# ravenprotocol/ravnest

Hardware: AMD Instinct MI355X
Metric: samples/sec (whole node), BERT-base MLM pretraining (higher is better)
Workload: dtype bf16; 1 GPU; model=bert-base, global_batch=128, seq_len=512, parallelism=dp1, reduce_factor=4, optimizer=fused_adam

## Files before the change

### ravnest_amd/csrc/bindings.cpp

```cpp
#include <torch/extension.h>

#include <vector>

std::vector<at::Tensor> layernorm_fwd(at::Tensor x, at::Tensor w,
                                      at::Tensor b, double eps);
std::vector<at::Tensor> layernorm_bwd(at::Tensor dy, at::Tensor x,
                                      at::Tensor w, at::Tensor mean,
                                      at::Tensor rstd);
std::vector<at::Tensor> layernorm_add_fwd(at::Tensor a, at::Tensor b,
                                          at::Tensor w, at::Tensor bias,
                                          double eps);
std::vector<at::Tensor> layernorm_mx_fwd(at::Tensor x, at::Tensor w,
                                         at::Tensor b, double eps);
at::Tensor bias_gelu_fwd(at::Tensor x, at::Tensor bias);
std::vector<at::Tensor> bias_gelu_mx_fwd(at::Tensor x, at::Tensor bias);
at::Tensor bias_gelu_bwd(at::Tensor dy, at::Tensor x, at::Tensor bias);
at::Tensor colsum_bf16(at::Tensor x);
std::vector<at::Tensor> bias_gelu_bwd_db(at::Tensor dy, at::Tensor x,
                                         at::Tensor bias);
std::vector<at::Tensor> batchnorm_fwd(at::Tensor x, at::Tensor w,
                                      at::Tensor b, at::Tensor running_mean,
                                      at::Tensor running_var, bool training,
                                      double momentum, double eps);
std::vector<at::Tensor> batchnorm_bwd(at::Tensor dy, at::Tensor x,
// ... 29 lines not shown
                   at::Tensor ws, c10::optional<at::Tensor> bias);
at::Tensor mx_gemm2(at::Tensor xq, at::Tensor xs, at::Tensor wq,
                    at::Tensor ws, c10::optional<at::Tensor> bias);
at::Tensor mx_scale_probe(at::Tensor a, at::Tensor b, at::Tensor sa,
                          at::Tensor sb);
at::Tensor softmax_fwd(at::Tensor x);
at::Tensor softmax_bwd(at::Tensor dy, at::Tensor y);
std::vector<at::Tensor> maxpool2d_fwd(at::Tensor x, long K, long S, long P);
at::Tensor maxpool2d_bwd(at::Tensor dy, at::Tensor idx, long H, long W,
                         long K, long S, long P);
at::Tensor avgpool2d_fwd(at::Tensor x, long K, long S, long P,
                         bool include_pad);
at::Tensor avgpool2d_bwd(at::Tensor dy, long H, long W, long K, long S,
                         long P, bool include_pad);
at::Tensor global_avgpool_fwd(at::Tensor x);
at::Tensor global_avgpool_bwd(at::Tensor dy, long H, long W);
std::vector<at::Tensor> emb2_ln_fwd(at::Tensor ids, at::Tensor word,
                                    at::Tensor pos, at::Tensor w,
                                    at::Tensor b, double eps);
at::Tensor emb2_add_fwd(at::Tensor ids, at::Tensor word, at::Tensor pos);
std::vector<at::Tensor> emb2_bwd(at::Tensor dx, at::Tensor ids, long V,
                                 long P);
std::vector<at::Tensor> dropout_fwd(at::Tensor x, double p, int64_t seed,
                                    c10::optional<at::Tensor> seed_buf);
at::Tensor dropout_bwd(at::Tensor dy, at::Tensor mask, double p);
std::vector<at::Tensor> dropout_add_ln_fwd(at::Tensor z, at::Tensor a,
                                           at::Tensor w, at::Tensor bias,
                                           double eps, double p, int64_t seed,
                                           c10::optional<at::Tensor> seed_buf);
std::vector<at::Tensor> dropout_add_ln_bwd(at::Tensor dy, at::Tensor s,
                                           at::Tensor w, at::Tensor mean,
                                           at::Tensor rstd,
                                           at::Tensor maskbits, double p);
std::vector<at::Tensor> ce_fwd(at::Tensor logits, at::Tensor targets,
                               int64_t ignore_index);
at::Tensor ce_bwd(at::Tensor logits, at::Tensor targets, at::Tensor lse,
                  at::Tensor gscale, int64_t ignore_index);
std::vector<at::Tensor> mlm_head_fwd(at::Tensor h, at::Tensor W,
                                     at::Tensor b, at::Tensor targets,
                                     int64_t ignore_index);
std::vector<at::Tensor> mlm_head_bwd(at::Tensor dloss, at::Tensor logits_c,
                                     at::Tensor lse, at::Tensor hc,
                                     at::Tensor tc, at::Tensor pos,
                                     at::Tensor count, at::Tensor W);
std::tuple<at::Tensor, long, long> mt_build_table(
    std::vector<at::Tensor> ps, std::vector<at::Tensor> gs,
    std::vector<at::Tensor> ms, std::vector<at::Tensor> vs,
    std::vector<at::Tensor> masters);
std::tuple<at::Tensor, long, long> grad_build_table(
    std::vector<at::Tensor> gs);
void grad_sqnorm(at::Tensor table, long nchunks, long esize,
                 at::Tensor partials, long offset);
void grad_norm_finalize(at::Tensor partials, long n, at::Tensor stats,
                        double max_norm,
                        c10::optional<at::Tensor> max_norm_buf);
void scale_mt(at::Tensor table, long nchunks, long esize, at::Tensor gstats);
void fused_adam_graph(at::Tensor table, long nchunks, long esize,
                      at::Tensor lr_buf, double b1, double b2, double eps,
                      double wd, at::Tensor step_buf,
                      c10::optional<at::Tensor> gstats);
void fused_adam_table(at::Tensor table, long nchunks, long esize, double lr,
                      double b1, double b2, double eps, double wd, double bc1,
                      double bc2, c10::optional<at::Tensor> gstats);
void fused_sgd_table(at::Tensor table, long nchunks, long esize, double lr,
                     double momentum, double wd, bool nesterov,
                     c10::optional<at::Tensor> gstats);
// ... 34 lines not shown
        "fused LayerNorm fwd + MX fp8 quantisation of y: y, mean, rstd, q, "
        "s (bf16 x, hidden % 32 == 0)");
  m.def("bias_gelu_fwd", &bias_gelu_fwd, "fused bias+GELU fwd");
  m.def("bias_gelu_mx_fwd", &bias_gelu_mx_fwd,
        "fused bias+GELU fwd + MX fp8 quantisation of y: y, q, s (bf16 x, "
        "last dim % 32 == 0)");
  m.def("bias_gelu_bwd", &bias_gelu_bwd, "fused bias+GELU bwd");
  m.def("colsum_bf16", &colsum_bf16, "column sum bf16 -> fp32");
  m.def("bias_gelu_bwd_db", &bias_gelu_bwd_db,
        "fused bias+GELU bwd with in-pass bias-grad column reduction");
  m.def("batchnorm_fwd", &batchnorm_fwd, "fused BatchNorm2d fwd (NCHW)");
  m.def("batchnorm_bwd", &batchnorm_bwd, "fused BatchNorm2d bwd (NCHW)");
  m.def("batchnorm_relu_launch_constants", &batchnorm_relu_launch_constants,
        "(grid cap, block size, bytes per lane) of the BN+ReLU elementwise "
        "kernels");
  m.def("batchnorm_relu_fwd", &batchnorm_relu_fwd,
        "fused BatchNorm2d + [residual add] + ReLU fwd (NCHW)", py::arg("x"),
        py::arg("residual"), py::arg("w"), py::arg("b"),
        py::arg("running_mean"), py::arg("running_var"),
        py::arg("training"), py::arg("momentum"), py::arg("eps"));
  m.def("batchnorm_relu_bwd", &batchnorm_relu_bwd,
        "fused BatchNorm2d + [residual add] + ReLU bwd: dx, dw, db[, dr]");
  m.def("dropout_fwd", &dropout_fwd, "philox dropout fwd (replayable)",
        py::arg("x"), py::arg("p"), py::arg("seed"),
        py::arg("seed_buf") = py::none());
  m.def("dropout_bwd", &dropout_bwd, "dropout bwd");
  m.def("dropout_add_ln_fwd", &dropout_add_ln_fwd,
        "fused dropout + residual add + LayerNorm fwd (bf16, bit mask)",
        py::arg("z"), py::arg("a"), py::arg("w"), py::arg("bias"),
        py::arg("eps"), py::arg("p"), py::arg("seed"),
        py::arg("seed_buf") = py::none());
  m.def("dropout_add_ln_bwd", &dropout_add_ln_bwd,
        "fused dropout + residual add + LayerNorm bwd: dx, dz, dw, db");
  m.def("conv2d_fwd", &conv2d_fwd,
        "implicit-GEMM MFMA conv fwd (bf16 NCHW)", py::arg("x"),
        py::arg("w"), py::arg("bias") = py::none(), py::arg("st") = 1,
        py::arg("pad") = 0, py::arg("relu") = false);
  m.def("conv2d_dgrad", &conv2d_dgrad, "implicit-GEMM MFMA conv dgrad");
  m.def("conv2d_wgrad", &conv2d_wgrad, "implicit-GEMM MFMA conv wgrad");
  m.def("gemm_nt_bf16", &gemm_nt_bf16,
        "bf16 MFMA GEMM x @ W^T (256^2 8-phase, fused bias/GELU epilogue)",
        py::arg("a"), py::arg("b"), py::arg("bias") = py::none(),
        py::arg("epi") = 0);
  m.def("gemm_wgrad_bf16", &gemm_wgrad_bf16,
        "split-K wgrad dW = dy^T @ x (tr16 transpose reads, fp32 atomics)");
  m.def("gemm_nt_bf16_rows", &gemm_nt_bf16_rows,
        "gemm_nt_bf16 into the caller's C (row stride C.size(1)), rows "
        "below a device-side int32 limit only; epi 0 or 1",
        py::arg("a"), py::arg("b"), py::arg("bias"), py::arg("epi"),
        py::arg("c"), py::arg("row_limit"));
  m.def("gemm_wgrad_bf16_rows", &gemm_wgrad_bf16_rows,
        "gemm_wgrad_bf16 over rows [0, round_up(min(*row_bound, M), 64))",
        py::arg("dy"), py::arg("x"), py::arg("row_bound"));
  m.def("mx_quant", &mx_quant,
        "bf16 -> MX fp8 (e4m3 + per-32 e8m0 scales)");
  m.def("mx_gemm", &mx_gemm, "MX fp8 GEMM: x @ W^T, 32x32x64 scaled MFMA",
        py::arg("x"), py::arg("xs"), py::arg("w"), py::arg("ws"),
        py::arg("bias") = py::none());
  m.def("mx_gemm2", &mx_gemm2,
        "LDS-staged MX fp8 GEMM (256^2 4-phase, scaled 32x32x64 MFMA)",
        py::arg("xq"), py::arg("xs"), py::arg("wq"), py::arg("ws"),
        py::arg("bias") = py::none());
  m.def("mx_scale_probe", &mx_scale_probe,
        "per-lane scale-byte semantics probe");
  m.def("softmax_fwd", &softmax_fwd, "standalone softmax fwd (last dim)");
  m.def("softmax_bwd", &softmax_bwd, "standalone softmax bwd");
// ... 81 lines not shown
```

### ravnest_amd/csrc/dropout_ln.hip

```cpp
#include <torch/extension.h>
#include <ATen/hip/HIPContext.h>

#include <cstdint>

#include "common.h"

namespace {

typedef unsigned int u32x2 __attribute__((ext_vector_type(2)));
typedef __bf16 hwbf16x2 __attribute__((ext_vector_type(2)));
typedef float f32x2 __attribute__((ext_vector_type(2)));

DEVINL unsigned int pack2(float lo, float hi) {
  const f32x2 v = {lo, hi};
  return __builtin_bit_cast(unsigned int,
                            __builtin_convertvector(v, hwbf16x2));
}
DEVINL u32x2 pack4(const float f[4]) {
  u32x2 r;
  r[0] = pack2(f[0], f[1]);
  r[1] = pack2(f[2], f[3]);
  return r;
}
DEVINL void unpack4(u32x2 v, float f[4]) {
// ... 139 lines not shown
      }
    }
    const float rstd = rsqrtf(wave_sum(s2) / H + eps);
    if (lane == 0) {
      mean_out[row] = mean;
      rstd_out[row] = rstd;
    }

#pragma unroll
    for (int k = 0; k < VPL; ++k) {
      const int g = lane + WAVE * k;
      if (FULL || g < G) {
        float wk[4], bk[4];
        if constexpr (HOIST) {
#pragma unroll
          for (int j = 0; j < 4; ++j) {
            wk[j] = wv[k][j];
            bk[j] = bv[k][j];
          }
        } else {
          load_p4(w + 4 * g, wk);
          load_p4(bias + 4 * g, bk);
        }
        float o[4];
#pragma unroll
        for (int j = 0; j < 4; ++j)
          o[j] = (sv[k][j] - mean) * rstd * wk[j] + bk[j];
        *reinterpret_cast<u32x2*>(y + base + 4 * g) = pack4(o);
      }
    }
  }
}

template <typename PT, int VPL, bool FULL>
__global__ __launch_bounds__(BWD_THREADS)
__attribute__((amdgpu_waves_per_eu(VPL <= 3 ? 4 : 1)))
void dropout_add_ln_bwd_kernel(
    const bf16_t* __restrict__ dy, const bf16_t* __restrict__ s,
    const PT* __restrict__ w, const float* __restrict__ mean,
    const float* __restrict__ rstd,
    const unsigned char* __restrict__ maskbits, bf16_t* __restrict__ dx,
    bf16_t* __restrict__ dz, float* __restrict__ part, int H, long N,
    float scale) {
  extern __shared__ float red[];
  constexpr bool HOIST = VPL <= 4;
  constexpr int PV = HOIST ? VPL : 1;
  const int lane = threadIdx.x & (WAVE - 1);
  const int wid = threadIdx.x / WAVE;
  const int wpb = blockDim.x / WAVE;
  const long nwaves = (long)gridDim.x * wpb;
  const int G = H >> 2;

  float wv[PV][4];
  if constexpr (HOIST) {
#pragma unroll
    for (int k = 0; k < VPL; ++k) {
      const int g = lane + WAVE * k;
      if (FULL || g < G) load_p4(w + 4 * g, wv[k]);
    }
  }
  float accw[VPL][4], accb[VPL][4];
#pragma unroll
  for (int k = 0; k < VPL; ++k)
#pragma unroll
    for (int j = 0; j < 4; ++j) accw[k][j] = accb[k][j] = 0.f;

  for (long row = (long)blockIdx.x * wpb + wid; row < N; row += nwaves) {
    const long base = row * H;
    u32x2 vd[VPL], vx[VPL];
    unsigned int mb[VPL];
#pragma unroll
    for (int k = 0; k < VPL; ++k) {
      const int g = lane + WAVE * k;
      if (FULL || g < G) {
        vd[k] = *reinterpret_cast<const u32x2*>(dy + base + 4 * g);
        vx[k] = *reinterpret_cast<const u32x2*>(s + base + 4 * g);
        mb[k] = maskbits[(base >> 3) + (g >> 1)];
      }
    }
    const float mu = mean[row], rs = rstd[row];

    float gv[VPL][4], xh[VPL][4];
    float c1 = 0.f, c2 = 0.f;
#pragma unroll
    for (int k = 0; k < VPL; ++k) {
      const int g = lane + WAVE * k;
      if (FULL || g < G) {
        float wk[4];
        if constexpr (HOIST) {
#pragma unroll
          for (int j = 0; j < 4; ++j) wk[j] = wv[k][j];
        } else {
          load_p4(w + 4 * g, wk);
        }
        float df[4], xf[4];
        unpack4(vd[k], df);
        unpack4(vx[k], xf);
#pragma unroll
        for (int j = 0; j < 4; ++j) {
          const float d = df[j];
          const float xhat = (xf[j] - mu) * rs;
          const float gg = d * wk[j];
          c1 += gg * xhat;
          c2 += gg;
          accw[k][j] += d * xhat;
          accb[k][j] += d;
          gv[k][j] = gg;
          xh[k][j] = xhat;
        }
      }
    }
    c1 = wave_sum(c1) / H;
    c2 = wave_sum(c2) / H;

#pragma unroll
    for (int k = 0; k < VPL; ++k) {
      const int g = lane + WAVE * k;
      if (FULL || g < G) {
        const unsigned int nib = mb[k] >> ((lane & 1) * 4);
        float o[4];
#pragma unroll
        for (int j = 0; j < 4; ++j)
          o[j] = rs * (gv[k][j] - xh[k][j] * c1 - c2);
        const u32x2 ox = pack4(o);
        unpack4(ox, o);
#pragma unroll
        for (int j = 0; j < 4; ++j)
          o[j] = ((nib >> j) & 1) ? o[j] * scale : 0.f;
        *reinterpret_cast<u32x2*>(dx + base + 4 * g) = ox;
        *reinterpret_cast<u32x2*>(dz + base + 4 * g) = pack4(o);
      }
    }
  }

  for (int t = 0; t < wpb; ++t) {
    if (wid == t) {
#pragma unroll
      for (int k = 0; k < VPL; ++k) {
        const int g = lane + WAVE * k;
        if (FULL || g < G) {
#pragma unroll
          for (int j = 0; j < 4; ++j) {
            const int c = 4 * g + j;
            if (t == 0) {
              red[c] = accw[k][j];
              red[H + c] = accb[k][j];
            } else {
              red[c] += accw[k][j];
              red[H + c] += accb[k][j];
            }
          }
        }
      }
    }
    __syncthreads();
  }
  float* prow = part + (long)blockIdx.x * 2 * H;
  for (int i = threadIdx.x; i < 2 * H; i += blockDim.x) prow[i] = red[i];
}

template <typename PT>
__global__ __launch_bounds__(1024) void dropout_add_ln_bwd_finalize_kernel(
    const float* __restrict__ part, PT* __restrict__ dw, PT* __restrict__ db,
    int H, int nparts) {
  __shared__ float tile[32][33];
  const int c = threadIdx.x & 31;
  const int sl = threadIdx.x >> 5;
  const int col = blockIdx.x * 32 + c;
  float acc = 0.f;
  if (col < 2 * H) {
#pragma unroll 4
    for (int q = sl; q < nparts; q += 32)
      acc += part[(long)q * 2 * H + col];
  }
  tile[sl][c] = acc;
  __syncthreads();
  if (sl == 0 && col < 2 * H) {
    float t = 0.f;
#pragma unroll
    for (int i = 0; i < 32; ++i) t += tile[i][c];
    if (col < H)
      store_p1(dw + col, t);
    else
      store_p1(db + (col - H), t);
  }
}

template <typename K>
int resident_blocks(K kernel, int threads, size_t lds) {
  int per_cu = 0;
  hipError_t e = hipOccupancyMaxActiveBlocksPerMultiprocessor(
      &per_cu, kernel, threads, lds);
  int dev = 0, cus = 0;
  if (e == hipSuccess) e = hipGetDevice(&dev);
  if (e == hipSuccess)
    e = hipDeviceGetAttribute(&cus, hipDeviceAttributeMultiprocessorCount,
                              dev);
  TORCH_CHECK(e == hipSuccess && per_cu > 0 && cus > 0,
              "dropout_add_ln: occupancy query failed");
  return per_cu * cus;
}

template <typename PT, int VPL, bool FULL>
int fwd_resident_blocks() {
  static const int n = resident_blocks(
      dropout_add_ln_fwd_kernel<PT, VPL, FULL>, FWD_THREADS, 0);
  return n;
}
template <typename PT, int VPL, bool FULL>
int bwd_resident_blocks() {
  static const int n = resident_blocks(
      dropout_add_ln_bwd_kernel<PT, VPL, FULL>, BWD_THREADS,
      2 * VPL * 256 * sizeof(float));
  return n;
}

bool aligned8(const at::Tensor& t) {
  return reinterpret_cast<uintptr_t>(t.data_ptr()) % 8 == 0;
}
bool aligned16(const at::Tensor& t) {
  return reinterpret_cast<uintptr_t>(t.data_ptr()) % 16 == 0;
}

void check_common(const at::Tensor& x, const at::Tensor& w, const char* op) {
  TORCH_CHECK(x.is_cuda() && x.is_contiguous() &&
                  x.scalar_type() == at::kBFloat16 && x.dim() >= 1,
              op, ": bf16 contiguous device activations only");
  const long H = x.size(-1);
  TORCH_CHECK(H % 8 == 0 && H <= MAX_H && H > 0, op,
              ": hidden size must be a multiple of 8, at most ", MAX_H);
  TORCH_CHECK(w.is_cuda() && w.is_contiguous() && w.numel() == H &&
                  (w.scalar_type() == at::kFloat ||
                   w.scalar_type() == at::kBFloat16) &&
                  aligned16(w),
              op, ": LN parameters must be fp32 or bf16 of size H");
}

}

#define DAL_FULL(PT, VPL, LAUNCH)                                           \
  do {                                                                      \
    if (full_ && vpl_ == VPL) { LAUNCH(PT, VPL, true); }                    \
    else { LAUNCH(PT, VPL, false); }                                        \
  } while (0)
#define DAL_DISPATCH_VPL(PT, LAUNCH)                                        \
  do {                                                                      \
// ... 29 lines not shown
  auto maskbits = at::empty({N * H / 8}, a.options().dtype(at::kByte));
  if (N == 0) return {y, s_out, mean, rstd, maskbits};
  const float scale = 1.0f / (1.0f - (float)p);
  auto stream = c10::hip::getCurrentHIPStreamMasqueradingAsCUDA().stream();
  const int wpb = FWD_THREADS / WAVE;

#define DAL_LAUNCH_FWD(PT, VPL, FULL)                                       \
  do {                                                                      \
    const long want = (N + wpb - 1) / wpb;                                  \
    const int cap = fwd_resident_blocks<PT, VPL, FULL>();                   \
    dim3 grid((unsigned)std::min<long>(want, cap));                         \
    hipLaunchKernelGGL((dropout_add_ln_fwd_kernel<PT, VPL, FULL>), grid,    \
                       dim3(FWD_THREADS), 0, stream,                        \
                       reinterpret_cast<const bf16_t*>(z.data_ptr()),       \
                       reinterpret_cast<const bf16_t*>(a.data_ptr()),       \
                       reinterpret_cast<const PT*>(w.data_ptr()),           \
                       reinterpret_cast<const PT*>(bias.data_ptr()),        \
                       reinterpret_cast<bf16_t*>(y.data_ptr()),             \
                       reinterpret_cast<bf16_t*>(s_out.data_ptr()),         \
                       mean.data_ptr<float>(), rstd.data_ptr<float>(),      \
                       maskbits.data_ptr<unsigned char>(), H, N,            \
                       (float)eps, (float)p, scale,                         \
                       (unsigned long long)seed, sb);                       \
  } while (0)

  if (w.scalar_type() == at::kFloat)
    DAL_DISPATCH_VPL(float, DAL_LAUNCH_FWD);
  else
    DAL_DISPATCH_VPL(bf16_t, DAL_LAUNCH_FWD);
  HIP_CHECK_LAST();
  return {y, s_out, mean, rstd, maskbits};
}

std::vector<at::Tensor> dropout_add_ln_bwd(at::Tensor dy, at::Tensor s,
                                           at::Tensor w, at::Tensor mean,
                                           at::Tensor rstd,
                                           at::Tensor maskbits, double p) {
  check_common(s, w, "dropout_add_ln_bwd");
  check_common(dy, w, "dropout_add_ln_bwd");
  TORCH_CHECK(dy.sizes() == s.sizes() && aligned8(dy) && aligned8(s));
  const int H = s.size(-1);
  const long N = s.numel() / H;
  TORCH_CHECK(mean.is_cuda() && mean.scalar_type() == at::kFloat &&
              mean.is_contiguous() && mean.numel() == N);
  TORCH_CHECK(rstd.is_cuda() && rstd.scalar_type() == at::kFloat &&
              rstd.is_contiguous() && rstd.numel() == N);
  TORCH_CHECK(maskbits.is_cuda() && maskbits.scalar_type() == at::kByte &&
              maskbits.is_contiguous() && maskbits.numel() == N * H / 8);
  TORCH_CHECK(p > 0.0 && p < 1.0, "dropout_add_ln_bwd: p must be in (0, 1)");
  auto dx = at::empty_like(s);
  auto dz = at::empty_like(s);
  auto dw = at::empty({H}, w.options());
  auto db = at::empty({H}, w.options());
  if (N == 0) {
    dw.zero_();
    db.zero_();
    return {dx, dz, dw, db};
  }
  const float scale = 1.0f / (1.0f - (float)p);
  auto stream = c10::hip::getCurrentHIPStreamMasqueradingAsCUDA().stream();
  const int wpb = BWD_THREADS / WAVE;
  const size_t lds = 2 * (size_t)H * sizeof(float);

#define DAL_LAUNCH_BWD(PT, VPL, FULL)                                       \
  do {                                                                      \
    const long want = (N + wpb - 1) / wpb;                                  \
    const int nparts =                                                      \
        (int)std::min<long>(want, bwd_resident_blocks<PT, VPL, FULL>());    \
    auto part = at::empty({nparts, 2 * H}, s.options().dtype(at::kFloat));  \
    hipLaunchKernelGGL((dropout_add_ln_bwd_kernel<PT, VPL, FULL>),          \
                       dim3(nparts),                                        \
                       dim3(BWD_THREADS), lds, stream,                      \
                       reinterpret_cast<const bf16_t*>(dy.data_ptr()),      \
                       reinterpret_cast<const bf16_t*>(s.data_ptr()),       \
                       reinterpret_cast<const PT*>(w.data_ptr()),           \
                       mean.data_ptr<float>(), rstd.data_ptr<float>(),      \
                       maskbits.data_ptr<unsigned char>(),                  \
                       reinterpret_cast<bf16_t*>(dx.data_ptr()),            \
                       reinterpret_cast<bf16_t*>(dz.data_ptr()),            \
                       part.data_ptr<float>(), H, N, scale);                \
    hipLaunchKernelGGL((dropout_add_ln_bwd_finalize_kernel<PT>),            \
                       dim3((2 * H + 31) / 32), dim3(1024), 0, stream,      \
                       part.data_ptr<float>(),                              \
                       reinterpret_cast<PT*>(dw.data_ptr()),                \
                       reinterpret_cast<PT*>(db.data_ptr()), H, nparts);    \
  } while (0)

  if (w.scalar_type() == at::kFloat)
    DAL_DISPATCH_VPL(float, DAL_LAUNCH_BWD);
  else
    DAL_DISPATCH_VPL(bf16_t, DAL_LAUNCH_BWD);
  HIP_CHECK_LAST();
  return {dx, dz, dw, db};
}
```

### ravnest_amd/csrc/gelu.hip

```cpp
#include <torch/extension.h>
#include <ATen/hip/HIPContext.h>

#include "common.h"
#include "mx_quant.h"

namespace {

template <typename PT>
DEVINL float load_pt(const PT* p);
template <>
DEVINL float load_pt<float>(const float* p) { return *p; }
template <>
DEVINL float load_pt<bf16_t>(const bf16_t* p) { return bf2f(*p); }

DEVINL float fast_tanh(float x) {
  const float t = __expf(2.f * x);
  return 1.f - 2.f * __builtin_amdgcn_rcpf(t + 1.f);
}

DEVINL float gelu_f(float x) {
  const float k = 0.7978845608028654f;
  float t = fast_tanh(k * (x + 0.044715f * x * x * x));
  return 0.5f * x * (1.f + t);
}

DEVINL float gelu_grad_f(float x) {
  const float k = 0.7978845608028654f;
  float x2 = x * x;
  float th = fast_tanh(k * (x + 0.044715f * x * x2));
  float sech2 = 1.f - th * th;
  return 0.5f * (1.f + th) + 0.5f * x * sech2 * k * (1.f + 3.f * 0.044715f * x2);
}

template <typename T, typename PT, bool MX = false>
// ... 91 lines not shown
                                        bf16_t* __restrict__ dx,
                                        float* __restrict__ db, int H,
                                        long N, long rows_per_chunk) {
  const int col = blockIdx.x * blockDim.x + threadIdx.x;
  const int chunk = blockIdx.y;
  if (col >= H) return;
  const float b = load_pt(bias + col);
  const long r0 = (long)chunk * rows_per_chunk;
  const long r1 = min(N, r0 + rows_per_chunk);
  float s = 0.f;
  long r = r0;
  for (; r + 8 <= r1; r += 8) {
    float xv[8], gv[8];
#pragma unroll
    for (int j = 0; j < 8; ++j) {
      xv[j] = bf2f(x[(r + j) * H + col]);
      gv[j] = bf2f(dy[(r + j) * H + col]);
    }
#pragma unroll
    for (int j = 0; j < 8; ++j) {
      const float d = gv[j] * gelu_grad_f(xv[j] + b);
      dx[(r + j) * H + col] = f2bf(d);
      s += d;
    }
  }
  for (; r < r1; ++r) {
    const float d = bf2f(dy[r * H + col]) * gelu_grad_f(bf2f(x[r * H + col]) + b);
    dx[r * H + col] = f2bf(d);
    s += d;
  }
  atomicAdd(&db[col], s);
}

}

static int grid_for(long work, int block) {
  long g = (work + block - 1) / block;
  return (int)std::min<long>(g, 2048);
}

static void check_bias_gelu(const at::Tensor& x, const at::Tensor& bias,
                            const char* who) {
  TORCH_CHECK(x.is_cuda() && x.is_contiguous() && x.dim() >= 1, who,
              ": x must be a contiguous GPU tensor");
  TORCH_CHECK(x.scalar_type() == at::kBFloat16 ||
                  x.scalar_type() == at::kFloat,
              who, ": x must be bf16 or fp32");
  TORCH_CHECK(bias.is_cuda() && bias.is_contiguous(), who,
              ": bias must be a contiguous GPU tensor");
  TORCH_CHECK(bias.scalar_type() == at::kFloat ||
                  (bias.scalar_type() == at::kBFloat16 &&
                   x.scalar_type() == at::kBFloat16),
              who, ": bias must be fp32, or bf16 with a bf16 x");
  TORCH_CHECK(bias.numel() >= 1 && x.size(-1) == bias.numel(), who,
              ": bias size mismatch");
}

at::Tensor bias_gelu_fwd(at::Tensor x, at::Tensor bias) {
  check_bias_gelu(x, bias, "bias_gelu_fwd");
  const int H = bias.numel();
  const long n = x.numel();
  auto y = at::empty_like(x);
  auto stream = c10::hip::getCurrentHIPStreamMasqueradingAsCUDA().stream();
  dim3 block(256);
  dim3 grid(grid_for(n / 8 + 1, 256));
  if (x.scalar_type() == at::kBFloat16 && bias.scalar_type() == at::kFloat) {
    hipLaunchKernelGGL((bias_gelu_fwd_kernel<bf16_t, float>), grid, block, 0,
                       stream, reinterpret_cast<const bf16_t*>(x.data_ptr()),
                       bias.data_ptr<float>(),
                       reinterpret_cast<bf16_t*>(y.data_ptr()), n, H);
  } else if (x.scalar_type() == at::kBFloat16) {
    hipLaunchKernelGGL((bias_gelu_fwd_kernel<bf16_t, bf16_t>), grid, block, 0,
                       stream, reinterpret_cast<const bf16_t*>(x.data_ptr()),
                       reinterpret_cast<const bf16_t*>(bias.data_ptr()),
                       reinterpret_cast<bf16_t*>(y.data_ptr()), n, H);
  } else {
    hipLaunchKernelGGL((bias_gelu_fwd_kernel<float, float>), grid, block, 0,
                       stream, x.data_ptr<float>(), bias.data_ptr<float>(),
                       y.data_ptr<float>(), n, H);
  }
  HIP_CHECK_LAST();
  return y;
}

std::vector<at::Tensor> bias_gelu_mx_fwd(at::Tensor x, at::Tensor bias) {
  check_bias_gelu(x, bias, "bias_gelu_mx_fwd");
  TORCH_CHECK(x.scalar_type() == at::kBFloat16,
              "bias_gelu_mx_fwd: x must be bf16");
  const int H = bias.numel();
  TORCH_CHECK(H % 32 == 0,
              "bias_gelu_mx_fwd: last dim % 32 == 0 required, got ", H);
  const long n = x.numel();
  auto y = at::empty_like(x);
  auto q = at::empty_like(x, x.options().dtype(at::kByte));
  auto s = at::empty({n / H, (long)(H / 32)}, x.options().dtype(at::kByte));
  if (n == 0) return {y, q, s};
  auto stream = c10::hip::getCurrentHIPStreamMasqueradingAsCUDA().stream();
  dim3 block(256);
  dim3 grid(grid_for(n / 8 + 1, 256));
  if (bias.scalar_type() == at::kFloat) {
    hipLaunchKernelGGL((bias_gelu_fwd_kernel<bf16_t, float, true>), grid,
                       block, 0, stream,
                       reinterpret_cast<const bf16_t*>(x.data_ptr()),
                       bias.data_ptr<float>(),
                       reinterpret_cast<bf16_t*>(y.data_ptr()), n, H,
                       q.data_ptr<unsigned char>(),
                       s.data_ptr<unsigned char>());
  } else {
    hipLaunchKernelGGL((bias_gelu_fwd_kernel<bf16_t, bf16_t, true>), grid,
                       block, 0, stream,
                       reinterpret_cast<const bf16_t*>(x.data_ptr()),
                       reinterpret_cast<const bf16_t*>(bias.data_ptr()),
                       reinterpret_cast<bf16_t*>(y.data_ptr()), n, H,
                       q.data_ptr<unsigned char>(),
                       s.data_ptr<unsigned char>());
  }
  HIP_CHECK_LAST();
  return {y, q, s};
}

at::Tensor bias_gelu_bwd(at::Tensor dy, at::Tensor x, at::Tensor bias) {
  check_bias_gelu(x, bias, "bias_gelu_bwd");
  TORCH_CHECK(dy.is_cuda() && dy.is_contiguous() &&
                  dy.scalar_type() == x.scalar_type() &&
                  dy.sizes() == x.sizes(),
              "bias_gelu_bwd: dy must match x in dtype and shape");
  const int H = bias.numel();
  const long n = x.numel();
  auto dx = at::empty_like(x);
// ... 81 lines not shown
```

### ravnest_amd/models/bert.py

```python
from __future__ import annotations

import torch
import torch.nn as nn

from ..ops import embedding_ln
from ..ops import (AttentionCoreQKV, Dropout, DropoutAddLayerNorm,
                   FusedLayerNorm, GELU, LinearGelu)
from ..ops.linear import make_linear


class BertConfig:
    def __init__(self, vocab_size=30522, hidden=768, layers=12, heads=12,
                 intermediate=3072, max_seq=512, type_vocab=2,
                 dropout=0.1, layer_norm_eps=1e-12):
        self.vocab_size = vocab_size
        self.hidden = hidden
        self.layers = layers
        self.heads = heads
        self.intermediate = intermediate
        self.max_seq = max_seq
        self.type_vocab = type_vocab
        self.dropout = dropout
        self.layer_norm_eps = layer_norm_eps

    @classmethod
    def base(cls, **kw):
        return cls(**kw)

    @classmethod
    def tiny(cls, **kw):
        d = dict(vocab_size=1024, hidden=128, layers=2, heads=2,
                 intermediate=256, max_seq=64)
        d.update(kw)
        return cls(**d)


class BertEmbeddings(nn.Module):
    _is_leaf_module = True

    def __init__(self, cfg: BertConfig):
        super().__init__()
        self.word = nn.Embedding(cfg.vocab_size, cfg.hidden)
        self.position = nn.Embedding(cfg.max_seq, cfg.hidden)
        self.ln = FusedLayerNorm(cfg.hidden, cfg.layer_norm_eps)
        self.drop = Dropout(cfg.dropout)
        self.register_buffer(
            "pos_ids", torch.arange(cfg.max_seq).unsqueeze(0),
            persistent=False)

    def forward(self, input_ids):
        if input_ids.is_cuda and self.word.weight.dtype == torch.bfloat16:
            y = embedding_ln(input_ids, self.word.weight,
                             self.position.weight, self.ln.weight,
                             self.ln.bias, self.ln.eps)
            return self.drop(y)
        S = input_ids.size(1)
        x = self.word(input_ids) + self.position(self.pos_ids[:, :S])
        return self.drop(self.ln(x))


class BertSelfAttention(nn.Module):

    def __init__(self, cfg: BertConfig):
        super().__init__()
        import os
        self.heads = cfg.heads
        self.head_dim = cfg.hidden // cfg.heads
        self.qkv = make_linear(cfg.hidden, 3 * cfg.hidden)
        exact = os.environ.get("RAVNEST_EXACT_ATTN_DROPOUT", "0") == "1"
        self.core = AttentionCoreQKV(
            causal=False, prob_dropout=cfg.dropout if exact else 0.0)
        self.out = make_linear(cfg.hidden, cfg.hidden)

    def forward(self, x, mask):
        qkv = self.qkv(x).unflatten(-1, (3, self.heads, self.head_dim))
        o = self.core(qkv, mask)
        return self.out(o)


class BertLayer(nn.Module):
    def __init__(self, cfg: BertConfig):
        super().__init__()
        self.attn = BertSelfAttention(cfg)
        self.ln1 = DropoutAddLayerNorm(cfg.hidden, cfg.layer_norm_eps,
                                       cfg.dropout)
        self.mlp_in = LinearGelu(cfg.hidden, cfg.intermediate)
        self.mlp_out = make_linear(cfg.intermediate, cfg.hidden)
        self.ln2 = DropoutAddLayerNorm(cfg.hidden, cfg.layer_norm_eps,
                                       cfg.dropout)

    def forward(self, x, mask):
        x = self.ln1(x, self.attn(x, mask))
        x = self.ln2(x, self.mlp_out(self.mlp_in(x)))
        return x


class BertMLMHead(nn.Module):
    def __init__(self, cfg: BertConfig):
        super().__init__()
        self.dense = make_linear(cfg.hidden, cfg.hidden)
        self.act = GELU()
        self.ln = FusedLayerNorm(cfg.hidden, cfg.layer_norm_eps)
        self.decoder = make_linear(cfg.hidden, cfg.vocab_size)

    def transform(self, x):
        return self.ln(self.act(self.dense(x)))

    def forward(self, x):
        return self.decoder(self.transform(x))


class BertForMLM(nn.Module):

    def __init__(self, cfg: BertConfig | None = None):
        super().__init__()
        self.cfg = cfg or BertConfig.base()
        self.embeddings = BertEmbeddings(self.cfg)
        self.layers = nn.ModuleList(
            [BertLayer(self.cfg) for _ in range(self.cfg.layers)])
        self.head = BertMLMHead(self.cfg)
        self.apply(self._init)

    @staticmethod
    def _init(m):
        from ..ops import Linear as _OpsLinear
        if isinstance(m, (nn.Linear, _OpsLinear)):
# ... 38 lines not shown
```

### ravnest_amd/ops/dropout_ln.py

```python
from __future__ import annotations

import os

import torch
import torch.nn as nn

from ._ext import get_ext
from .dropout import dropout
from .layernorm import add_layer_norm

_MAX_FUSED_H = 2048


class _DropoutAddLayerNormFn(torch.autograd.Function):
    @staticmethod
    def forward(ctx, a, z, weight, bias, eps, p):
        ext = get_ext(required=True)
        from . import rng
        seed = int(torch.randint(0, 2**62, (1,)).item())
        y, s, mean, rstd, maskbits = ext.dropout_add_ln_fwd(
            z, a, weight, bias, eps, p, seed,
            rng.device_seed_counter(a.device))
        ctx.save_for_backward(s, weight, mean, rstd, maskbits)
        ctx.p = p
        return y

    @staticmethod
    def backward(ctx, dy):
        s, weight, mean, rstd, maskbits = ctx.saved_tensors
        ext = get_ext(required=True)
        dx, dz, dw, db = ext.dropout_add_ln_bwd(
            dy.contiguous(), s, weight, mean, rstd, maskbits, ctx.p)
        need = ctx.needs_input_grad
        return (dx if need[0] else None, dz if need[1] else None,
                dw if need[2] else None, db if need[3] else None,
                None, None)


def _fusable(a, z, weight, bias) -> bool:
    H = a.shape[-1]
    return (a.is_cuda and z.is_cuda
            and a.dtype == torch.bfloat16 and z.dtype == torch.bfloat16
            and a.shape == z.shape
            and H % 8 == 0 and H <= _MAX_FUSED_H
            and weight.dtype == bias.dtype
            and weight.dtype in (torch.float32, torch.bfloat16))


def dropout_add_layer_norm(a, z, weight, bias, eps: float = 1e-12,
                           p: float = 0.1, training: bool = True,
                           fused: bool = True):
    if fused and training and 0.0 < p < 1.0 and _fusable(a, z, weight, bias):
        return _DropoutAddLayerNormFn.apply(
            a.contiguous(), z.contiguous(), weight, bias, eps, p)
    return add_layer_norm(a, dropout(z, p, training), weight, bias, eps)


class DropoutAddLayerNorm(nn.Module):
    _is_leaf_module = True

    def __init__(self, hidden: int, eps: float = 1e-12, p: float = 0.1):
        super().__init__()
        self.weight = nn.Parameter(torch.ones(hidden))
        self.bias = nn.Parameter(torch.zeros(hidden))
        self.eps = eps
        self.p = p
        self.fused = os.environ.get("RAVNEST_FUSED_DROPOUT_LN", "1") != "0"

    def forward(self, a, z):
        return dropout_add_layer_norm(a, z, self.weight, self.bias, self.eps,
                                      self.p, self.training, self.fused)
```

Before: 1896 samples/s.

## Fuse output-linear bias grad into dropout-add-LN backward and vectorize bias-GELU fwd

The linear layers feeding the dropout+residual+LayerNorm blocks now detach their bias, and its gradient (column sum of dz) is accumulated inside the fused LN backward kernel, in registers or LDS per wave, then reduced in the finalize kernel. This drops the separate bias-gradient reduction over dz. A separate change adds a vectorized, row-unrolled bias+GELU forward kernel. In exchange, the bias-grad path uses more LDS, which may lower occupancy, and bias gradients are summed from bf16-rounded dz values.

```diff
diff --git a/ravnest_amd/csrc/bindings.cpp b/ravnest_amd/csrc/bindings.cpp
--- a/ravnest_amd/csrc/bindings.cpp
+++ b/ravnest_amd/csrc/bindings.cpp
@@ -85,6 +85,9 @@
                                            at::Tensor w, at::Tensor mean,
                                            at::Tensor rstd,
                                            at::Tensor maskbits, double p);
+std::vector<at::Tensor> dropout_add_ln_bwd_dzsum(
+    at::Tensor dy, at::Tensor s, at::Tensor w, at::Tensor mean,
+    at::Tensor rstd, at::Tensor maskbits, double p, bool dzsum_bf16);
 std::vector<at::Tensor> ce_fwd(at::Tensor logits, at::Tensor targets,
                                int64_t ignore_index);
 at::Tensor ce_bwd(at::Tensor logits, at::Tensor targets, at::Tensor lse,
@@ -185,6 +188,9 @@
         py::arg("seed_buf") = py::none());
   m.def("dropout_add_ln_bwd", &dropout_add_ln_bwd,
         "fused dropout + residual add + LayerNorm bwd: dx, dz, dw, db");
+  m.def("dropout_add_ln_bwd_dzsum", &dropout_add_ln_bwd_dzsum,
+        "dropout_add_ln_bwd and dzsum = dz.sum(0), fp32 or bf16: dx, dz, dw, "
+        "db, dzsum");
   m.def("conv2d_fwd", &conv2d_fwd,
         "implicit-GEMM MFMA conv fwd (bf16 NCHW)", py::arg("x"),
         py::arg("w"), py::arg("bias") = py::none(), py::arg("st") = 1,
diff --git a/ravnest_amd/csrc/dropout_ln.hip b/ravnest_amd/csrc/dropout_ln.hip
--- a/ravnest_amd/csrc/dropout_ln.hip
+++ b/ravnest_amd/csrc/dropout_ln.hip
@@ -195,7 +195,7 @@
   }
 }
 
-template <typename PT, int VPL, bool FULL>
+template <typename PT, int VPL, bool FULL, bool DZS = false>
 __global__ __launch_bounds__(BWD_THREADS)
 __attribute__((amdgpu_waves_per_eu(VPL <= 3 ? 4 : 1)))
 void dropout_add_ln_bwd_kernel(
@@ -206,6 +206,10 @@
     bf16_t* __restrict__ dz, float* __restrict__ part, int H, long N,
     float scale) {
   extern __shared__ float red[];
+  constexpr int NS = DZS ? 3 : 2;
+  constexpr bool ZLDS = DZS && VPL <= 4;
+  constexpr bool ZREG = DZS && !ZLDS;
+  constexpr int ZV = ZREG ? VPL : 1;
   constexpr bool HOIST = VPL <= 4;
   constexpr int PV = HOIST ? VPL : 1;
   const int lane = threadIdx.x & (WAVE - 1);
@@ -227,6 +231,22 @@
   for (int k = 0; k < VPL; ++k)
 #pragma unroll
     for (int j = 0; j < 4; ++j) accw[k][j] = accb[k][j] = 0.f;
+  float accz[ZV][4];
+  if constexpr (ZREG) {
+#pragma unroll
+    for (int k = 0; k < VPL; ++k)
+#pragma unroll
+      for (int j = 0; j < 4; ++j) accz[k][j] = 0.f;
+  }
+  float* zrow = red + 2 * H + wid * H;
+  if constexpr (ZLDS) {
+#pragma unroll
+    for (int k = 0; k < VPL; ++k) {
+      const int g = lane + WAVE * k;
+      if (FULL || g < G)
+        *reinterpret_cast<f32x4*>(zrow + 4 * g) = f32x4{0.f, 0.f, 0.f, 0.f};
+    }
+  }
 
   for (long row = (long)blockIdx.x * wpb + wid; row < N; row += nwaves) {
     const long base = row * H;
@@ -291,7 +311,19 @@
         for (int j = 0; j < 4; ++j)
           o[j] = ((nib >> j) & 1) ? o[j] * scale : 0.f;
         *reinterpret_cast<u32x2*>(dx + base + 4 * g) = ox;
-        *reinterpret_cast<u32x2*>(dz + base + 4 * g) = pack4(o);
+        const u32x2 oz = pack4(o);
+        *reinterpret_cast<u32x2*>(dz + base + 4 * g) = oz;
+        if constexpr (DZS) unpack4(oz, o);
+        if constexpr (ZREG) {
+#pragma unroll
+          for (int j = 0; j < 4; ++j) accz[k][j] += o[j];
+        }
+        if constexpr (ZLDS) {
+          f32x4 zs = *reinterpret_cast<f32x4*>(zrow + 4 * g);
+#pragma unroll
+          for (int j = 0; j < 4; ++j) zs[j] += o[j];
+          *reinterpret_cast<f32x4*>(zrow + 4 * g) = zs;
+        }
       }
     }
   }
@@ -308,9 +340,11 @@
             if (t == 0) {
               red[c] = accw[k][j];
               red[H + c] = accb[k][j];
+              if constexpr (ZREG) red[2 * H + c] = accz[k][j];
             } else {
               red[c] += accw[k][j];
               red[H + c] += accb[k][j];
+              if constexpr (ZREG) red[2 * H + c] += accz[k][j];
             }
           }
         }
@@ -318,34 +352,45 @@
     }
     __syncthreads();
   }
-  float* prow = part + (long)blockIdx.x * 2 * H;
-  for (int i = threadIdx.x; i < 2 * H; i += blockDim.x) prow[i] = red[i];
-}
-
-template <typename PT>
+  float* prow = part + (long)blockIdx.x * NS * H;
+  if constexpr (ZLDS) {
+    for (int i = threadIdx.x; i < 2 * H; i += blockDim.x) prow[i] = red[i];
+    for (int i = threadIdx.x; i < H; i += blockDim.x) {
+      float t = 0.f;
+      for (int w = 0; w < wpb; ++w) t += red[2 * H + w * H + i];
+      prow[2 * H + i] = t;
+    }
+  } else {
+    for (int i = threadIdx.x; i < NS * H; i += blockDim.x) prow[i] = red[i];
+  }
+}
+
+template <typename PT, typename ZT>
 __global__ __launch_bounds__(1024) void dropout_add_ln_bwd_finalize_kernel(
     const float* __restrict__ part, PT* __restrict__ dw, PT* __restrict__ db,
-    int H, int nparts) {
+    ZT* __restrict__ dzs, int H, int nparts, int ns) {
   __shared__ float tile[32][33];
   const int c = threadIdx.x & 31;
   const int sl = threadIdx.x >> 5;
   const int col = blockIdx.x * 32 + c;
   float acc = 0.f;
-  if (col < 2 * H) {
+  if (col < ns * H) {
 #pragma unroll 4
     for (int q = sl; q < nparts; q += 32)
-      acc += part[(long)q * 2 * H + col];
+      acc += part[(long)q * ns * H + col];
   }
   tile[sl][c] = acc;
   __syncthreads();
-  if (sl == 0 && col < 2 * H) {
+  if (sl == 0 && col < ns * H) {
     float t = 0.f;
 #pragma unroll
     for (int i = 0; i < 32; ++i) t += tile[i][c];
     if (col < H)
       store_p1(dw + col, t);
+    else if (col < 2 * H)
+      store_p1(db + (col - H), t);
     else
-      store_p1(db + (col - H), t);
+      store_p1(dzs + (col - 2 * H), t);
   }
 }
 
@@ -370,11 +415,15 @@
       dropout_add_ln_fwd_kernel<PT, VPL, FULL>, FWD_THREADS, 0);
   return n;
 }
-template <typename PT, int VPL, bool FULL>
+template <int VPL, bool DZS>
+constexpr size_t bwd_lds_floats(int H) {
+  return (size_t)(!DZS ? 2 : VPL <= 4 ? 2 + BWD_THREADS / WAVE : 3) * H;
+}
+template <typename PT, int VPL, bool FULL, bool DZS>
 int bwd_resident_blocks() {
   static const int n = resident_blocks(
-      dropout_add_ln_bwd_kernel<PT, VPL, FULL>, BWD_THREADS,
-      2 * VPL * 256 * sizeof(float));
+      dropout_add_ln_bwd_kernel<PT, VPL, FULL, DZS>, BWD_THREADS,
+      bwd_lds_floats<VPL, DZS>(VPL * 256) * sizeof(float));
   return n;
 }
 
@@ -470,10 +519,9 @@
   return {y, s_out, mean, rstd, maskbits};
 }
 
-std::vector<at::Tensor> dropout_add_ln_bwd(at::Tensor dy, at::Tensor s,
-                                           at::Tensor w, at::Tensor mean,
-                                           at::Tensor rstd,
-                                           at::Tensor maskbits, double p) {
+static std::vector<at::Tensor> dropout_add_ln_bwd_impl(
+    at::Tensor dy, at::Tensor s, at::Tensor w, at::Tensor mean,
+    at::Tensor rstd, at::Tensor maskbits, double p, int zs) {
   check_common(s, w, "dropout_add_ln_bwd");
   check_common(dy, w, "dropout_add_ln_bwd");
   TORCH_CHECK(dy.sizes() == s.sizes() && aligned8(dy) && aligned8(s));
@@ -490,25 +538,37 @@
   auto dz = at::empty_like(s);
   auto dw = at::empty({H}, w.options());
   auto db = at::empty({H}, w.options());
+  at::Tensor dzs;
+  if (zs)
+    dzs = at::empty({H}, w.options().dtype(zs == 1 ? at::kFloat
+                                                   : at::kBFloat16));
   if (N == 0) {
     dw.zero_();
     db.zero_();
+    if (zs) {
+      dzs.zero_();
+      return {dx, dz, dw, db, dzs};
+    }
     return {dx, dz, dw, db};
   }
   const float scale = 1.0f / (1.0f - (float)p);
   auto stream = c10::hip::getCurrentHIPStreamMasqueradingAsCUDA().stream();
   const int wpb = BWD_THREADS / WAVE;
-  const size_t lds = 2 * (size_t)H * sizeof(float);
-
-#define DAL_LAUNCH_BWD(PT, VPL, FULL)                                       \
+  const int ns = zs ? 3 : 2;
+  const long want = (N + wpb - 1) / wpb;
+  at::Tensor part;
+  int nparts = 0;
+
+#define DAL_LAUNCH_BWD_MAIN(PT, VPL, FULL, DZS)                             \
   do {                                                                      \
-    const long want = (N + wpb - 1) / wpb;                                  \
-    const int nparts =                                                      \
-        (int)std::min<long>(want, bwd_resident_blocks<PT, VPL, FULL>());    \
-    auto part = at::empty({nparts, 2 * H}, s.options().dtype(at::kFloat));  \
-    hipLaunchKernelGGL((dropout_add_ln_bwd_kernel<PT, VPL, FULL>),          \
+    nparts = (int)std::min<long>(                                           \
+        want, bwd_resident_blocks<PT, VPL, FULL, DZS>());                   \
+    part = at::empty({nparts, ns * H}, s.options().dtype(at::kFloat));      \
+    hipLaunchKernelGGL((dropout_add_ln_bwd_kernel<PT, VPL, FULL, DZS>),     \
                        dim3(nparts),                                        \
-                       dim3(BWD_THREADS), lds, stream,                      \
+                       dim3(BWD_THREADS),                                   \
+                       (bwd_lds_floats<VPL, DZS>(H)) * sizeof(float),       \
+                       stream,                                              \
                        reinterpret_cast<const bf16_t*>(dy.data_ptr()),      \
                        reinterpret_cast<const bf16_t*>(s.data_ptr()),       \
                        reinterpret_cast<const PT*>(w.data_ptr()),           \
@@ -517,11 +577,21 @@
                        reinterpret_cast<bf16_t*>(dx.data_ptr()),            \
                        reinterpret_cast<bf16_t*>(dz.data_ptr()),            \
                        part.data_ptr<float>(), H, N, scale);                \
-    hipLaunchKernelGGL((dropout_add_ln_bwd_finalize_kernel<PT>),            \
-                       dim3((2 * H + 31) / 32), dim3(1024), 0, stream,      \
-                       part.data_ptr<float>(),                              \
-                       reinterpret_cast<PT*>(dw.data_ptr()),                \
-                       reinterpret_cast<PT*>(db.data_ptr()), H, nparts);    \
+  } while (0)
+#define DAL_LAUNCH_BWD_FIN(PT, ZT)                                          \
+  hipLaunchKernelGGL((dropout_add_ln_bwd_finalize_kernel<PT, ZT>),          \
+                     dim3((ns * H + 31) / 32), dim3(1024), 0, stream,       \
+                     part.data_ptr<float>(),                                \
+                     reinterpret_cast<PT*>(dw.data_ptr()),                  \
+                     reinterpret_cast<PT*>(db.data_ptr()),                  \
+                     zs ? reinterpret_cast<ZT*>(dzs.data_ptr()) : nullptr,  \
+                     H, nparts, ns)
+#define DAL_LAUNCH_BWD(PT, VPL, FULL)                                       \
+  do {                                                                      \
+    if (zs) DAL_LAUNCH_BWD_MAIN(PT, VPL, FULL, true);                       \
+    else DAL_LAUNCH_BWD_MAIN(PT, VPL, FULL, false);                         \
+    if (zs == 2) DAL_LAUNCH_BWD_FIN(PT, bf16_t);                            \
+    else DAL_LAUNCH_BWD_FIN(PT, float);                                     \
   } while (0)
 
   if (w.scalar_type() == at::kFloat)
@@ -529,5 +599,20 @@
   else
     DAL_DISPATCH_VPL(bf16_t, DAL_LAUNCH_BWD);
   HIP_CHECK_LAST();
+  if (zs) return {dx, dz, dw, db, dzs};
   return {dx, dz, dw, db};
 }
+
+std::vector<at::Tensor> dropout_add_ln_bwd(at::Tensor dy, at::Tensor s,
+                                           at::Tensor w, at::Tensor mean,
+                                           at::Tensor rstd,
+                                           at::Tensor maskbits, double p) {
+  return dropout_add_ln_bwd_impl(dy, s, w, mean, rstd, maskbits, p, 0);
+}
+
+std::vector<at::Tensor> dropout_add_ln_bwd_dzsum(
+    at::Tensor dy, at::Tensor s, at::Tensor w, at::Tensor mean,
+    at::Tensor rstd, at::Tensor maskbits, double p, bool dzsum_bf16) {
+  return dropout_add_ln_bwd_impl(dy, s, w, mean, rstd, maskbits, p,
+                                 dzsum_bf16 ? 2 : 1);
+}
diff --git a/ravnest_amd/csrc/gelu.hip b/ravnest_amd/csrc/gelu.hip
--- a/ravnest_amd/csrc/gelu.hip
+++ b/ravnest_amd/csrc/gelu.hip
@@ -1,5 +1,8 @@
 #include <torch/extension.h>
 #include <ATen/hip/HIPContext.h>
+
+#include <cstdint>
+#include <cstdlib>
 
 #include "common.h"
 #include "mx_quant.h"
@@ -157,11 +160,101 @@
   atomicAdd(&db[col], s);
 }
 
+constexpr int VEC_UNROLL = 4;
+
+template <typename PT>
+DEVINL void load_bias8(const PT* p, float b[8]) {
+#pragma unroll
+  for (int j = 0; j < 8; ++j) b[j] = load_pt(p + j);
+}
+
+template <typename PT, bool MX>
+__global__ __launch_bounds__(256) void bias_gelu_fwd_vec_kernel(
+    const bf16_t* __restrict__ x, const PT* __restrict__ bias,
+    bf16_t* __restrict__ y, long N, int G, long rows_per_sweep,
+    unsigned char* __restrict__ q, unsigned char* __restrict__ qs) {
+  const long t = (long)blockIdx.x * blockDim.x + threadIdx.x;
+  if (t >= rows_per_sweep * G) return;
+  const int cg = (int)(t % G);
+  float b[8];
+  load_bias8(bias + 8 * cg, b);
+
+  auto one = [&](long r, bf16x8 v) {
+    const long i = r * G + cg;
+    bf16x8 o;
+#pragma unroll
+    for (int j = 0; j < 8; ++j)
+      o[j] = (short)f2us(gelu_f(us2f((unsigned short)v[j]) + b[j]));
+    *reinterpret_cast<bf16x8*>(y + i * 8) = o;
+    if constexpr (MX) {
+      float yq[8];
+#pragma unroll
+      for (int j = 0; j < 8; ++j) yq[j] = us2f((unsigned short)o[j]);
+      mx_quant8(yq, q + i * 8, qs + (i >> 2), threadIdx.x);
+    }
+  };
+
+  long r = t / G;
+  for (; r + (VEC_UNROLL - 1) * rows_per_sweep < N;
+       r += VEC_UNROLL * rows_per_sweep) {
+    bf16x8 v[VEC_UNROLL];
+#pragma unroll
+    for (int u = 0; u < VEC_UNROLL; ++u)
+      v[u] = *reinterpret_cast<const bf16x8*>(
+          x + ((r + u * rows_per_sweep) * G + cg) * 8);
+#pragma unroll
+    for (int u = 0; u < VEC_UNROLL; ++u) one(r + u * rows_per_sweep, v[u]);
+  }
+  for (; r < N; r += rows_per_sweep)
+    one(r, *reinterpret_cast<const bf16x8*>(x + (r * G + cg) * 8));
+}
+
 }
 
 static int grid_for(long work, int block) {
   long g = (work + block - 1) / block;
   return (int)std::min<long>(g, 2048);
+}
+
+static bool gelu_v1() {
+  const char* e = std::getenv("RAVNEST_GELU_V1");
+  return e && e[0] == '1';
+}
+
+static bool aligned16(const at::Tensor& t) {
+  return reinterpret_cast<uintptr_t>(t.data_ptr()) % 16 == 0;
+}
+
+template <bool MX>
+static bool bias_gelu_fwd_vec(const at::Tensor& x, const at::Tensor& bias,
+                              at::Tensor& y, unsigned char* q,
+                              unsigned char* qs) {
+  const int H = (int)bias.numel();
+  if (gelu_v1() || x.scalar_type() != at::kBFloat16 || (H & 7) ||
+      x.numel() == 0 || !aligned16(x) || !aligned16(y))
+    return false;
+  const int G = H >> 3;
+  const long N = x.numel() / H;
+  const int blocks = grid_for(N * G, 256);
+  const long rows_per_sweep = std::min<long>(N, (long)blocks * 256 / G);
+  if (rows_per_sweep == 0) return false;
+  auto stream = c10::hip::getCurrentHIPStreamMasqueradingAsCUDA().stream();
+  if (bias.scalar_type() == at::kFloat)
+    hipLaunchKernelGGL((bias_gelu_fwd_vec_kernel<float, MX>), dim3(blocks),
+                       dim3(256), 0, stream,
+                       reinterpret_cast<const bf16_t*>(x.data_ptr()),
+                       bias.data_ptr<float>(),
+                       reinterpret_cast<bf16_t*>(y.data_ptr()), N, G,
+                       rows_per_sweep, q, qs);
+  else
+    hipLaunchKernelGGL((bias_gelu_fwd_vec_kernel<bf16_t, MX>), dim3(blocks),
+                       dim3(256), 0, stream,
+                       reinterpret_cast<const bf16_t*>(x.data_ptr()),
+                       reinterpret_cast<const bf16_t*>(bias.data_ptr()),
+                       reinterpret_cast<bf16_t*>(y.data_ptr()), N, G,
+                       rows_per_sweep, q, qs);
+  HIP_CHECK_LAST();
+  return true;
 }
 
 static void check_bias_gelu(const at::Tensor& x, const at::Tensor& bias,
@@ -186,6 +279,7 @@
   const int H = bias.numel();
   const long n = x.numel();
   auto y = at::empty_like(x);
+  if (bias_gelu_fwd_vec<false>(x, bias, y, nullptr, nullptr)) return y;
   auto stream = c10::hip::getCurrentHIPStreamMasqueradingAsCUDA().stream();
   dim3 block(256);
   dim3 grid(grid_for(n / 8 + 1, 256));
@@ -220,6 +314,9 @@
   auto q = at::empty_like(x, x.options().dtype(at::kByte));
   auto s = at::empty({n / H, (long)(H / 32)}, x.options().dtype(at::kByte));
   if (n == 0) return {y, q, s};
+  if (bias_gelu_fwd_vec<true>(x, bias, y, q.data_ptr<unsigned char>(),
+                              s.data_ptr<unsigned char>()))
+    return {y, q, s};
   auto stream = c10::hip::getCurrentHIPStreamMasqueradingAsCUDA().stream();
   dim3 block(256);
   dim3 grid(grid_for(n / 8 + 1, 256));
diff --git a/ravnest_amd/models/bert.py b/ravnest_amd/models/bert.py
--- a/ravnest_amd/models/bert.py
+++ b/ravnest_amd/models/bert.py
@@ -1,12 +1,23 @@
 from __future__ import annotations
+
+import os
 
 import torch
 import torch.nn as nn
+import torch.nn.functional as F
 
 from ..ops import embedding_ln
 from ..ops import (AttentionCoreQKV, Dropout, DropoutAddLayerNorm,
                    FusedLayerNorm, GELU, LinearGelu)
 from ..ops.linear import make_linear
+
+
+def _plain_biased_linear(lin) -> bool:
+    return type(lin) is nn.Linear and lin.bias is not None
+
+
+def _linear_bias_downstream(lin, x):
+    return F.linear(x, lin.weight, lin.bias.detach())
 
 
 class BertConfig:
@@ -72,9 +83,11 @@
             causal=False, prob_dropout=cfg.dropout if exact else 0.0)
         self.out = make_linear(cfg.hidden, cfg.hidden)
 
-    def forward(self, x, mask):
+    def forward(self, x, mask, out_bias_downstream: bool = False):
         qkv = self.qkv(x).unflatten(-1, (3, self.heads, self.head_dim))
         o = self.core(qkv, mask)
+        if out_bias_downstream:
+            return _linear_bias_downstream(self.out, o)
         return self.out(o)
 
 
@@ -88,10 +101,25 @@
         self.mlp_out = make_linear(cfg.intermediate, cfg.hidden)
         self.ln2 = DropoutAddLayerNorm(cfg.hidden, cfg.layer_norm_eps,
                                        cfg.dropout)
+        self.fused_bias_grad = \
+            os.environ.get("RAVNEST_FUSED_BIAS_GRAD", "1") != "0"
+
+    def _bias_downstream(self, ln, a, lin) -> bool:
+        return (self.fused_bias_grad and torch.is_tensor(a)
+                and _plain_biased_linear(lin) and ln.takes_zbias(a, lin))
 
     def forward(self, x, mask):
-        x = self.ln1(x, self.attn(x, mask))
-        x = self.ln2(x, self.mlp_out(self.mlp_in(x)))
+        if self._bias_downstream(self.ln1, x, self.attn.out):
+            x = self.ln1(x, self.attn(x, mask, out_bias_downstream=True),
+                         zbias=self.attn.out.bias)
+        else:
+            x = self.ln1(x, self.attn(x, mask))
+        if self._bias_downstream(self.ln2, x, self.mlp_out):
+            x = self.ln2(x, _linear_bias_downstream(self.mlp_out,
+                                                    self.mlp_in(x)),
+                         zbias=self.mlp_out.bias)
+        else:
+            x = self.ln2(x, self.mlp_out(self.mlp_in(x)))
         return x
 
 
diff --git a/ravnest_amd/ops/dropout_ln.py b/ravnest_amd/ops/dropout_ln.py
--- a/ravnest_amd/ops/dropout_ln.py
+++ b/ravnest_amd/ops/dropout_ln.py
@@ -14,7 +14,7 @@
 
 class _DropoutAddLayerNormFn(torch.autograd.Function):
     @staticmethod
-    def forward(ctx, a, z, weight, bias, eps, p):
+    def forward(ctx, a, z, weight, bias, eps, p, zbias):
         ext = get_ext(required=True)
         from . import rng
         seed = int(torch.randint(0, 2**62, (1,)).item())
@@ -23,18 +23,25 @@
             rng.device_seed_counter(a.device))
         ctx.save_for_backward(s, weight, mean, rstd, maskbits)
         ctx.p = p
+        ctx.zbias_dtype = None if zbias is None else zbias.dtype
         return y
 
     @staticmethod
     def backward(ctx, dy):
         s, weight, mean, rstd, maskbits = ctx.saved_tensors
         ext = get_ext(required=True)
-        dx, dz, dw, db = ext.dropout_add_ln_bwd(
-            dy.contiguous(), s, weight, mean, rstd, maskbits, ctx.p)
         need = ctx.needs_input_grad
+        dzsum = None
+        if need[6]:
+            dx, dz, dw, db, dzsum = ext.dropout_add_ln_bwd_dzsum(
+                dy.contiguous(), s, weight, mean, rstd, maskbits, ctx.p,
+                ctx.zbias_dtype == torch.bfloat16)
+        else:
+            dx, dz, dw, db = ext.dropout_add_ln_bwd(
+                dy.contiguous(), s, weight, mean, rstd, maskbits, ctx.p)
         return (dx if need[0] else None, dz if need[1] else None,
                 dw if need[2] else None, db if need[3] else None,
-                None, None)
+                None, None, dzsum)
 
 
 def _fusable(a, z, weight, bias) -> bool:
@@ -47,12 +54,23 @@
             and weight.dtype in (torch.float32, torch.bfloat16))
 
 
+def _zbias_ok(zbias, H) -> bool:
+    return (zbias.is_cuda and zbias.shape == (H,)
+            and zbias.dtype in (torch.float32, torch.bfloat16))
+
+
 def dropout_add_layer_norm(a, z, weight, bias, eps: float = 1e-12,
                            p: float = 0.1, training: bool = True,
-                           fused: bool = True):
+                           fused: bool = True, zbias=None):
     if fused and training and 0.0 < p < 1.0 and _fusable(a, z, weight, bias):
-        return _DropoutAddLayerNormFn.apply(
-            a.contiguous(), z.contiguous(), weight, bias, eps, p)
+        if zbias is None or _zbias_ok(zbias, a.shape[-1]):
+            return _DropoutAddLayerNormFn.apply(
+                a.contiguous(), z.contiguous(), weight, bias, eps, p, zbias)
+    if zbias is not None:
+        raise RuntimeError(
+            "dropout_add_layer_norm: zbias needs the fused path (training, "
+            "0 < p < 1, CUDA bf16 activations, a fp32 or bf16 bias of the "
+            "hidden size)")
     return add_layer_norm(a, dropout(z, p, training), weight, bias, eps)
 
 
@@ -67,6 +85,17 @@
         self.p = p
         self.fused = os.environ.get("RAVNEST_FUSED_DROPOUT_LN", "1") != "0"
 
-    def forward(self, a, z):
+    def takes_zbias(self, a, lin) -> bool:
+        b = lin.bias
+        return (self.fused and self.training and 0.0 < self.p < 1.0
+                and torch.is_tensor(a) and b is not None
+                and lin.weight.dtype == a.dtype
+                and lin.weight.shape[0] == a.shape[-1]
+                and not torch.is_autocast_enabled()
+                and _fusable(a, a, self.weight, self.bias)
+                and _zbias_ok(b, a.shape[-1]))
+
+    def forward(self, a, z, zbias=None):
         return dropout_add_layer_norm(a, z, self.weight, self.bias, self.eps,
-                                      self.p, self.training, self.fused)
+                                      self.p, self.training, self.fused,
+                                      zbias)
```

After: 1918 samples/s (median of 6 runs). 1.01x the previous value.
